# kylc/optik

Hardware: AMD Instinct MI355X
Metric: random-restart IK solves/sec (Panda 7-DoF, 1e-6 tol) (higher is better)
Workload: dtype f64

## Files before the change

### include/optik_hip.h

```cpp
#ifndef OPTIK_HIP_H
#define OPTIK_HIP_H

#include <stdint.h>

#ifdef __cplusplus
extern "C" {
#endif

#define OPTIK_HIP_MAX_DOF 16

enum {
    OPTIK_HIP_OK = 0,
    OPTIK_HIP_EINVAL = -1,
    OPTIK_HIP_EUNSUPPORTED = -2,
    OPTIK_HIP_ENODEVICE = -3,
    OPTIK_HIP_ENOMEM = -4
};

enum { OPTIK_JOINT_FIXED = 0, OPTIK_JOINT_REVOLUTE = 1, OPTIK_JOINT_PRISMATIC = 2 };

enum {
    OPTIK_RES_FAILURE = -1,
    OPTIK_RES_ROUNDOFF_LIMITED = -4,
    OPTIK_RES_FORCED_STOP = -5,
// ... 195 lines not shown
                           const double *d_targets, const double *d_x0, int32_t T, const double *ee_offset7,
                           uint64_t restart_begin, uint64_t restart_end, double deadline_s,
                           int32_t K, double min_dist, const optik_hip_ik_solutions_outputs *out, void *stream);

#define OPTIK_HIP_PATH_MAX_RESTARTS 4096
typedef struct optik_hip_ik_path_outputs {
    double *d_x;
    double *d_f;
    uint64_t *d_idx;
    double *d_key;
    double *d_step;
    double *d_last;
} optik_hip_ik_path_outputs;
int optik_hip_ik_path(optik_hip_chain *chain, const optik_solver_config *cfg, const double *d_targets,
                      const double *d_x0, int32_t P, int32_t L, const double *ee_offset7, uint64_t restart_begin,
                      uint64_t restart_end, uint32_t flags, double deadline_s, double max_step,
                      const optik_hip_ik_path_outputs *out, void *stream);

int optik_hip_set_option(const char *name, long long value);
long long optik_hip_get_option(const char *name);

int optik_hip_ik_host(optik_hip_chain *chain, const optik_solver_config *cfg,
                      const double *targets, const double *x0, int32_t T, const double *ee_offset7,
                      uint64_t restart_begin, uint64_t restart_end, uint32_t flags,
                      double deadline_s, double *win_x, double *win_f, uint64_t *win_idx,
                      double *win_key);

int optik_hip_probe(int32_t op, const double *a, const double *b, int64_t count, double *out);
int optik_hip_probe_math(int32_t op, const double *poses7, int64_t count, double *out);

typedef struct optik_hip_launch_info {
    int32_t grid, block, lds_bytes, tiles;
    float kernel_ms;
} optik_hip_launch_info;
void optik_hip_set_timing(optik_hip_chain *chain, int32_t enabled);
int optik_hip_last_launch(const optik_hip_chain *chain, optik_hip_launch_info *info);
int optik_hip_timing_mean(optik_hip_chain *chain, double *mean_ms, int32_t *count);
int optik_hip_phase_profile(optik_hip_chain *chain, unsigned long long *out8);

#ifdef __cplusplus
}
#endif
#endif
```

### optik_amd/_native.py

```python
from __future__ import annotations

import ctypes as C
import math
import os

_HERE = os.path.dirname(os.path.abspath(__file__))
LIB_PATH = os.path.join(_HERE, "csrc", "liboptik_amd.so")
if os.environ.get("OPTIK_AMD_LIB"):
    LIB_PATH = os.path.abspath(os.environ["OPTIK_AMD_LIB"])

MAX_DOF = 8
IK_EARLY_EXIT = 1
IK_FIND_ANY = 2
IK_RESTART_MAJOR = 4
UINT64_MAX = 0xFFFFFFFFFFFFFFFF

RES_FAILURE, RES_ROUNDOFF, RES_FORCED_STOP, RES_ITER_CAP = -1, -4, -5, -100
RES_STOPVAL, RES_FTOL, RES_XTOL = 2, 3, 4
RANGE_SINGLE_INCLUSIVE, RANGE_NEW_INCLUSIVE = 0, 1


class OptikHipError(RuntimeError):
    pass

# ... 25 lines not shown
                ("d_key", C.c_void_p)]


MAX_SOLUTIONS = 256
MAX_SOLUTION_RESTARTS = 1 << 22


def check_solutions_args(k, min_dist):
    if isinstance(k, bool) or int(k) != k or not 1 <= int(k) <= MAX_SOLUTIONS:
        raise ValueError(f"k must be an integer in 1..{MAX_SOLUTIONS}, got {k!r}")
    min_dist = float(min_dist)
    if not (min_dist >= 0.0 and min_dist != float("inf")):
        raise ValueError(f"min_dist must be finite and >= 0, got {min_dist!r}")
    return int(k), min_dist


class IkPathOutputs(C.Structure):
    _fields_ = [("d_x", C.c_void_p), ("d_f", C.c_void_p), ("d_idx", C.c_void_p), ("d_key", C.c_void_p),
                ("d_step", C.c_void_p), ("d_last", C.c_void_p)]


PATH_MAX_RESTARTS = 4096


def check_max_step(max_step):
    max_step = float(max_step)
    if not max_step >= 0.0:
        raise ValueError(f"max_step must be >= 0 (+inf: no limit), got {max_step!r}")
    return max_step


class LaunchInfo(C.Structure):
    _fields_ = [("grid", C.c_int32), ("block", C.c_int32), ("lds_bytes", C.c_int32),
                ("tiles", C.c_int32), ("kernel_ms", C.c_float)]


_lib = None


def lib():
    global _lib
    if _lib is not None:
        return _lib
    if not os.path.exists(LIB_PATH):
        raise OptikHipError(
            f"{LIB_PATH} is missing: build it with `python -c 'import __graft_entry__ as g; "
            "g.build()'` (hipcc --offload-arch=gfx950).  optik_amd has no CPU fallback.")
    L = C.CDLL(LIB_PATH, mode=C.RTLD_GLOBAL)
    vp, dp, ip = C.c_void_p, C.POINTER(C.c_double), C.POINTER(C.c_int32)
    L.optik_hip_device_count.restype = C.c_int
    L.optik_hip_set_option.argtypes = [C.c_char_p, C.c_longlong]
    L.optik_hip_get_option.argtypes = [C.c_char_p]
    L.optik_hip_get_option.restype = C.c_longlong
    L.optik_hip_last_error.restype = C.c_char_p
    L.optik_hip_chain_create.argtypes = [dp, dp, ip, C.c_int32, dp, dp, C.c_int32, C.POINTER(vp)]
    L.optik_hip_chain_destroy.argtypes = [vp]
    L.optik_hip_chain_num_positions.argtypes = [vp]
    L.optik_hip_chain_set_range_rule.argtypes = [vp, C.c_int32]
    L.optik_hip_chain_range_rule.argtypes = [vp]
    L.optik_hip_eval_batch.argtypes = [vp, C.POINTER(SolverConfigC), dp, dp, vp, C.c_int64, vp, vp, vp]
    L.optik_hip_fk_batch.argtypes = [vp, dp, vp, C.c_int64, vp, vp, vp]
    L.optik_hip_seed_batch.argtypes = [vp, C.c_uint64, C.c_int64, vp, vp]
    L.optik_hip_manip_batch.argtypes = [vp, dp, vp, C.c_int64, vp, vp, vp]
    ip = C.POINTER(C.c_int32)
    L.optik_hip_chain_set_collision_model.argtypes = [vp, ip, dp, dp, C.c_int32, ip, C.c_int32, C.c_double]
    L.optik_hip_chain_set_world.argtypes = [vp, dp, C.c_int32, dp, C.c_int32]
    L.optik_hip_chain_set_world_grid.argtypes = [vp, dp, C.c_double, C.c_int32, C.c_int32, C.c_int32, vp]
# ... 256 lines not shown
```

### optik_amd/csrc/ik_batch_ops.hip

```cpp
#include "diff_ik_lp.hpp"
#include "ik_host.hpp"
#include "ik_jacobian.hpp"

using namespace optik;
using namespace optik::host;
using namespace optik::hostparams;

namespace {

struct EvalLaunch {
    const ChainDev *chain;
    EvalParams ep;
    double target[7];
    const double *q;
    long long B;
    double *f;
    double *g;
};

template <int N, bool TIP>
__global__ __launch_bounds__(256) void eval_batch_kernel(const EvalLaunch a) {
    __shared__ ChainDev sch;
    stage_chain(sch, a.chain);
    const Pose target = load_pose(a.target);
// ... 130 lines not shown
                ++qi;
            } else if (a.types[j] == OPTIK_JOINT_PRISMATIC) {
                const double d = a.q[(size_t)qi * a.B + b];
                local.t = V3{a.axis[j][0] * d, a.axis[j][1] * d, a.axis[j][2] * d};
                ++qi;
            }
            const Pose jt = pose_mul(load_pose(a.origin[j]), local);
            state = pose_mul(state, jt);
        }
        const Pose ee = pose_mul(state, load_pose(a.ee_offset));
        const double p[7] = {ee.t.x, ee.t.y, ee.t.z, ee.q.i, ee.q.j, ee.q.k, ee.q.w};
#pragma unroll
        for (int i = 0; i < 7; ++i) a.pose[(size_t)i * a.B + b] = p[i];
    }
}

struct SeedLaunch {
    uint32_t key[8];
    double lb[MAX_DOF];
    double scale[MAX_DOF];
    unsigned long long first;
    long long count;
    double *q;
};

template <int N>
__global__ __launch_bounds__(256) void seed_batch_kernel(const SeedLaunch a) {
    for (long long b = (long long)blockIdx.x * blockDim.x + threadIdx.x; b < a.count;
         b += (long long)gridDim.x * blockDim.x) {
        double q[N];
        restart_seed<N>(a.key, a.lb, a.scale, a.first + (unsigned long long)b, q);
#pragma unroll
        for (int i = 0; i < N; ++i) a.q[(size_t)i * a.count + b] = q[i];
    }
}

__global__ void probe_kernel(int op, const double *a, const double *b, long long count, double *out) {
    for (long long i = (long long)blockIdx.x * blockDim.x + threadIdx.x; i < count;
         i += (long long)gridDim.x * blockDim.x) {
        double r = 0.0, s, c;
        switch (op) {
        case 0: r = a[i] / b[i]; break;
        case 1: r = __builtin_sqrt(a[i]); break;
        case 2: sincos_dev(a[i], s, c); r = s; break;
        case 3: sincos_dev(a[i], s, c); r = c; break;
        default: r = atan2_q1(a[i], b[i]); break;
        }
        out[i] = r;
    }
}

__global__ void probe_math_kernel(int op, const double *poses, long long count, double *out, int stride) {
    for (long long i = (long long)blockIdx.x * blockDim.x + threadIdx.x; i < count;
         i += (long long)gridDim.x * blockDim.x) {
        const Pose X = load_pose(poses + i * 7);
        double *o = out + i * stride;
        const V3 w = so3_log(X.q);
        if (op == 0) { o[0] = w.x; o[1] = w.y; o[2] = w.z; continue; }
        const RotTerms rt = rot_terms(w);
        const M3 Jr = so3_right_jacobian(rt);
        if (op == 1) {
            for (int r = 0; r < 3; ++r) for (int c = 0; c < 3; ++c) o[r * 3 + c] = Jr.m[r][c];
        } else if (op == 2) {
            const V3 lin = se3_log_linear(rt, X.t);
            o[0] = lin.x; o[1] = lin.y; o[2] = lin.z; o[3] = w.x; o[4] = w.y; o[5] = w.z;
        } else {
            const M3 Q = se3_q_matrix(rt, X.t, Jr);
            for (int r = 0; r < 3; ++r)
                for (int c = 0; c < 3; ++c) {
                    o[r * 6 + c] = Jr.m[r][c];
                    o[r * 6 + 3 + c] = Q.m[r][c];
                    o[(r + 3) * 6 + c] = 0.0;
                    o[(r + 3) * 6 + 3 + c] = Jr.m[r][c];
                }
        }
    }
}

const char *const kPrismaticJacobianMsg =
    "joint_jacobian: prismatic joints are not implemented (the reference panics: kinematics.rs:185 todo!())";

}

extern "C" {

int optik_hip_eval_batch(const optik_hip_chain *ch, const optik_solver_config *cfg, const double *target7,
                         const double *ee_offset7, const double *d_q, int64_t B, double *d_f, double *d_g,
                         void *stream) {
    if (!ch || !cfg || !target7 || !d_q || !d_f || B < 0) return fail(OPTIK_HIP_EINVAL, "bad argument");
    if (B == 0) return 0;
    if (ch->prismatic)
        return fail(OPTIK_HIP_EUNSUPPORTED,
                    "prismatic joints: only forward kinematics is available (the reference's Jacobian panics, kinematics.rs:185)");
    BIND_DEVICE(ch);
    if (ch->wide) {
        WideBatchLaunch w;
        std::memset(&w, 0, sizeof w);
        w.chain = ch->wdev;
        make_eval_params(cfg->linear_weight, cfg->angular_weight, ee_offset7, w.ep);
        std::memcpy(w.target, target7, sizeof w.target);
        w.q = d_q; w.B = B; w.f = d_f; w.g = d_g;
        HIP_TRY(wide_batch_launch(0, grid_for(ch, B, 256, 8), (hipStream_t)stream, w));
        return 0;
    }
    EvalLaunch a;
    a.chain = ch->dev;
    make_eval_params(cfg->linear_weight, cfg->angular_weight, ee_offset7, a.ep);
    std::memcpy(a.target, target7, sizeof a.target);
    a.q = d_q; a.B = B; a.f = d_f; a.g = d_g;
    const int grid = grid_for(ch, B, 256, 8);
#define CALL(NN, TT) hipLaunchKernelGGL((eval_batch_kernel<NN, TT>), dim3(grid), dim3(256), 0, (hipStream_t)stream, a)
    OPTIK_DISPATCH(ch, CALL);
#undef CALL
    HIP_TRY(hipGetLastError());
    return 0;
}
// ... 138 lines not shown
```

### optik_amd/csrc/ik_capi.hip

```cpp
#include <algorithm>
#include <cstdio>
#include <cstdlib>
#include <vector>

#include "ik_host.hpp"

using namespace optik;
using namespace optik::host;
using namespace optik::hostparams;

namespace optik {
namespace host {

thread_local std::string g_err;

static int solve_kernel_from(const char *e) {
    if (!e) return SK_AUTO;
    if (!std::strcmp(e, "quad")) return SK_QUAD;
    if (!std::strcmp(e, "lane64")) return SK_LANE64;
    if (!std::strcmp(e, "general")) return SK_GENERAL;
    return SK_AUTO;
}
Options &opt() {
    static Options o = [] {
// ... 160 lines not shown
    ch->fs_clean = sl.fs_clean_after;
    ch->clean_stream = stream;
}

static int solve_locked(optik_hip_chain *ch, const optik_solver_config *cfg, const double *d_targets,
                        const double *d_x0, int32_t T, const double *ee_offset7, uint64_t restart_begin,
                        uint64_t restart_end, uint32_t flags, double deadline_s, const optik_hip_ik_outputs *out,
                        bool want_sel, bool need_x, bool need_f, hipStream_t stream, bool claim_request,
                        bool *claim_armed, SolvedLaunch *sl) {
    if (!ch || !cfg || !d_targets || !d_x0 || !out || T < 1) return fail(OPTIK_HIP_EINVAL, "bad argument");
    if (restart_end <= restart_begin) return fail(OPTIK_HIP_EINVAL, "empty restart range");
    const int mode = cfg->solution_mode;
    if (mode < OPTIK_MODE_QUALITY || mode > OPTIK_MODE_CONDITION)
        return fail(OPTIK_HIP_EINVAL,
                    "solution_mode must be 1 (Quality), 2 (Speed), 3 (Manipulability) or 4 (Condition)");
    const bool manip = mode == OPTIK_MODE_MANIPULABILITY || mode == OPTIK_MODE_CONDITION;
    const bool coll = ch && ch->coll_S > 0;
    const uint64_t R = restart_end - restart_begin;
    if (restart_end > 1 || restart_begin > 0)
        for (int k = 0; k < ch->n; ++k)
            if (std::isnan(ch->scale[k]))
                return fail(OPTIK_HIP_EINVAL, "random restarts need finite joint limits (reference: random_range panics)");
    if (ch->prismatic)
        return fail(OPTIK_HIP_EUNSUPPORTED,
                    "prismatic joints: only forward kinematics is available (the reference's Jacobian panics, kinematics.rs:185)");

    PlanIn in{};
    in.n = ch->n; in.wide = ch->wide; in.cus = ch->num_cus;
    in.T = T; in.R = R; in.flags = flags; in.mode = mode; in.coll = coll;
    in.solve_kernel = opt().solve_kernel; in.wide_form = opt().wide_form;
    in.claim_request = claim_request; in.have_claim_block = ch->hw_claim != nullptr;
    in.lane_waves = lane_solve_waves_per_cu(); in.quad_waves = quad_solve_waves_per_cu(ch->n);
    in.latency_waves = 4; in.wide_waves = 8;
    const LaunchPlan plan = plan_launch(in);
    if (plan.error == PLAN_TOO_MANY_TILES)
        return fail(OPTIK_HIP_EINVAL, "too many restarts / targets in one launch (2^24 or more selection tiles)");
    const bool early = plan.early, wide_lds = plan.solver == WIDE_LDS, widek = wide_lds || plan.solver == WIDE_HBM;
    const size_t cols = (size_t)plan.cols;

    BIND_DEVICE(ch);
    if (ch->claim_pending && stream != nullptr) { HIP_TRY(hipStreamSynchronize(nullptr)); ch->claim_pending = false; }
    HIP_TRY(ch->tile_recs.reserve((size_t)plan.n_tiles));
    if (!ch->queue) { HIP_TRY(hipMalloc(&ch->queue, sizeof(unsigned long long))); ch->queue_clean = false; }
    if (stream != ch->clean_stream) { ch->queue_clean = false; ch->fs_clean = 0; }
    if (!ch->queue_clean) HIP_TRY(hipMemsetAsync(ch->queue, 0, sizeof(unsigned long long), stream));
    ch->queue_clean = false;
    size_t fs_clean_after = ch->fs_clean;
    if (early) {
        if ((size_t)T > ch->first_success.capacity()) ch->fs_clean = 0;
        HIP_TRY(ch->first_success.reserve((size_t)T));
        if (ch->fs_clean < (size_t)T)
            HIP_TRY(hipMemsetAsync(ch->first_success.get(), 0xff, sizeof(unsigned long long) * (size_t)T, stream));
        fs_clean_after = std::max(ch->fs_clean, (size_t)T);
        ch->fs_clean = 0;
    }
    double *px = out->d_x, *pf = out->d_f, *pk = nullptr;
    need_x = need_x || (want_sel && (manip || coll));
    if (want_sel) {
        const bool need_xf = (!px || !pf) && (need_x || need_f);
        if (cols > ch->tmp_key.capacity()) {
            HIP_TRY(ch->tmp_x.reset());
            HIP_TRY(ch->tmp_f.reset());
            HIP_TRY(ch->tmp_key.reserve(cols));
        }
        if (need_xf) {
            HIP_TRY(ch->tmp_x.reserve(ch->tmp_key.capacity() * (size_t)ch->n));
            HIP_TRY(ch->tmp_f.reserve(ch->tmp_key.capacity()));
        }
        pk = ch->tmp_key.get();
        if (!px && need_x) px = ch->tmp_x.get();
        if (!pf && need_f) pf = ch->tmp_f.get();
    }

    if (widek && !ch->wide) {
        fill_wide_chain(ch->whost, &ch->host.origin[0][0], &ch->host.axis[0][0], ch->host.lb, ch->host.ub, ch->n, ch->tip,
                        ch->scale);
        HIP_TRY(upload_table(&ch->wdev, ch->whost));
    }
    if (plan.solver == WIDE_HBM) HIP_TRY(ch->wide_ws.reserve(wide_ws_doubles_per_wave() * (size_t)plan.grid));

    SolveLaunch a;
    std::memset(&a, 0, sizeof a);
    a.chain = ch->dev;
    make_eval_params(cfg->linear_weight, cfg->angular_weight, ee_offset7, a.ep);
    fill_solve_params(cfg, a.sp, opt().stop_x_legacy != 0);
    std::memcpy(a.key, ch->key, sizeof a.key);
    std::memcpy(a.scale, ch->scale, sizeof a.scale);
    a.wq.next_item = ch->queue;
    a.wq.total_items = (unsigned long long)cols;
    a.wq.n_restarts = R;
    a.wq.restart_begin = restart_begin;
    a.wq.targets = d_targets;
    a.wq.x0 = d_x0;
    a.wq.first_success = early ? ch->first_success.get() : nullptr;
    a.wq.find_any = plan.find_any ? 1 : 0;
    a.wq.restart_major = plan.restart_major ? 1 : 0;
    a.wq.n_targets = (unsigned long long)T;
    a.wq.quality = plan.quality;
    a.wq.lanes = plan.lanes;
    a.wq.out_x = px;
    a.wq.out_f = pf;
    a.wq.out_key = pk;
    a.wq.out_status = out->d_status;
    a.wq.out_evals = out->d_evals;
#ifdef OPTIK_PROFILE
    if (!ch->prof) HIP_TRY(hipMalloc(&ch->prof, 8 * sizeof(unsigned long long)));
    HIP_TRY(hipMemsetAsync(ch->prof, 0, 8 * sizeof(unsigned long long), stream));
    a.wq.prof = ch->prof;
#endif
    if (deadline_s > 0.0) {
        const double khz = ch->wall_clock_khz > 0 ? (double)ch->wall_clock_khz : 100000.0;
        a.deadline_ticks = (unsigned long long)(deadline_s * khz * 1e3);
        if (a.deadline_ticks == 0) a.deadline_ticks = 1;
    }
    if (plan.arm_claim) {
        a.wq.claim = ch->hw_claim;
        a.wq.claim_seq = ++ch->claim_seq;
        if (claim_armed) *claim_armed = true;
        if (stream == nullptr) ch->claim_pending = true;
    }
    const int ev_slot = ch->ev_count % optik_hip_chain::EV_POOL;
    if (ch->timing) {
        if (!ch->ev0[ev_slot]) { HIP_TRY(hipEventCreate(&ch->ev0[ev_slot])); HIP_TRY(hipEventCreate(&ch->ev1[ev_slot])); }
        HIP_TRY(hipEventRecord(ch->ev0[ev_slot], stream));
    }
    int lds = 0;
    if (widek) {
        WideSolveLaunch w;
        std::memset(&w, 0, sizeof w);
        w.chain = ch->wdev;
        w.ep = a.ep; w.sp = a.sp; w.wq = a.wq;
        std::memcpy(w.key, ch->key, sizeof w.key);
        w.deadline_ticks = a.deadline_ticks;
        w.ws = ch->wide_ws.get();
        lds = wide_lds ? wide_lds_bytes() : (int)sizeof(WideChainDev);
        HIP_TRY(wide_solve_launch(plan.grid, stream, w, wide_lds, opt().wide_form != 2));
    } else if (plan.solver == LANE) {
        HIP_TRY(lane_solve_launch(ch->n, ch->tip, plan.grid, stream, a, &lds));
    } else {
        HIP_TRY(quad_solve_launch(ch->n, ch->tip, plan.grid, stream, a, &lds, plan.solver == QUAD_LATENCY));
    }
    HIP_TRY(hipGetLastError());
    if (ch->timing) { HIP_TRY(hipEventRecord(ch->ev1[ev_slot], stream)); ch->ev_count += 1; }
    if (manip && pk)
        if (int rc = manip_key_launch(ch, mode, ee_offset7, px, pk, cols, stream)) return rc;
    if (coll && pk)
        if (int rc = collision_key_launch(ch, ee_offset7, px, pk, cols, stream)) return rc;
    ch->last.grid = plan.grid; ch->last.block = WAVE; ch->last.lds_bytes = lds; ch->last.tiles = plan.n_tiles;

    sl->px = px; sl->pf = pf; sl->pk = pk;
    sl->R = R;
    sl->tiles_per_target = plan.tiles_per_target;
    sl->cols = cols;
    sl->fs_clean_after = fs_clean_after;
    sl->early = early;
    return 0;
}

static int ik_batch_locked(optik_hip_chain *ch, const optik_solver_config *cfg, const double *d_targets,
                           const double *d_x0, int32_t T, const double *ee_offset7, uint64_t restart_begin,
                           uint64_t restart_end, uint32_t flags, double deadline_s, const optik_hip_ik_outputs *out,
                           void *stream_v, bool claim_request = false, bool *claim_armed = nullptr) {
    if (claim_armed) *claim_armed = false;
    if (!out) return fail(OPTIK_HIP_EINVAL, "bad argument");
    hipStream_t stream = (hipStream_t)stream_v;
    const bool want_win = out->d_win_x || out->d_win_f || out->d_win_idx || out->d_win_key;
    SolvedLaunch sl;
    if (int rc = solve_locked(ch, cfg, d_targets, d_x0, T, ee_offset7, restart_begin, restart_end, flags, deadline_s,
                              out, want_win, out->d_win_x != nullptr, out->d_win_f != nullptr, stream, claim_request,
                              claim_armed, &sl))
        return rc;
    BIND_DEVICE(ch);
    if (want_win) {
        SelectLaunch s;
        std::memset(&s, 0, sizeof s);
        s.out_key = sl.pk; s.out_x = sl.px; s.out_f = sl.pf;
        s.tile_recs = ch->tile_recs.get();
        s.tiles_per_target = (int)sl.tiles_per_target;
        s.tile = SEL_TILE;
        s.n = ch->n;
        s.restart_begin = restart_begin;
// ... 103 lines not shown
        PathSelectLaunch s;
        std::memset(&s, 0, sizeof s);
        s.out_key = sl.pk; s.out_x = sl.px; s.out_f = sl.pf;
        s.seed = seed;
        s.carry = ch->path_carry.get();
        s.last = l + 1 == L ? out->d_last : nullptr;
        s.n = n;
        s.filter = filter ? 1 : 0;
        s.max_step = max_step;
        s.restart_begin = restart_begin;
        s.n_restarts = sl.R;
        s.ld = sl.cols;
        s.x = out->d_x ? out->d_x + w * (size_t)n : nullptr;
        s.f = out->d_f ? out->d_f + w : nullptr;
        s.idx = out->d_idx ? (unsigned long long *)out->d_idx + w : nullptr;
        s.key = out->d_key ? out->d_key + w : nullptr;
        s.step = out->d_step ? out->d_step + w : nullptr;
        s.reset_queue = ch->queue;
        s.reset_fs = sl.early ? ch->first_success.get() : nullptr;
        HIP_TRY(path_select_launch(s, P, stream));
        words_put_back(ch, sl, stream);
    }
    return 0;
}

static int *option_slot(const char *name) {
    Options &o = opt();
    if (!name) return nullptr;
    if (!std::strcmp(name, "solve_kernel")) return &o.solve_kernel;
    if (!std::strcmp(name, "wide_form")) return &o.wide_form;
    if (!std::strcmp(name, "range_rule")) return &o.range_rule;
    if (!std::strcmp(name, "stop_x_legacy")) return &o.stop_x_legacy;
    if (!std::strcmp(name, "grid_cap")) return &o.grid_cap;
    return nullptr;
}
int optik_hip_set_option(const char *name, long long value) {
    int *slot = option_slot(name);
    if (!slot) return fail(OPTIK_HIP_EINVAL, "unknown option");
    if (slot == &opt().grid_cap && (value < 0 || value > 0x7fffffffll))
        return fail(OPTIK_HIP_EINVAL, "grid_cap must be >= 0 (0: the device's cap)");
    *slot = (int)value;
    return 0;
}
long long optik_hip_get_option(const char *name) {
    const int *slot = option_slot(name);
    return slot ? (long long)*slot : -1;
}

int optik_hip_ik_host(optik_hip_chain *ch, const optik_solver_config *cfg, const double *targets,
                      const double *x0, int32_t T, const double *ee_offset7, uint64_t restart_begin,
                      uint64_t restart_end, uint32_t flags, double deadline_s, double *win_x, double *win_f,
                      uint64_t *win_idx, double *win_key) {
    if (!ch || !cfg || !targets || !x0 || T < 1) return fail(OPTIK_HIP_EINVAL, "bad argument");
    std::lock_guard<std::mutex> host_lock(ch->host_mu);
    BIND_DEVICE(ch);
    const int n = ch->n;
    const size_t n_in = (size_t)(7 + n) * (size_t)T, n_out = (size_t)(n + 3) * (size_t)T;
    std::unique_lock<std::mutex> launch_lock(ch->mu);
    if (n_in + n_out > ch->hw_dev.capacity() || 2 * (n_in + n_out) > ch->hw_pin.capacity()) {
        if (ch->claim_pending) { (void)hipStreamSynchronize(nullptr); ch->claim_pending = false; }
        HIP_TRY(ch->hw_dev.reserve(n_in + n_out));
        HIP_TRY(ch->hw_pin.reserve(2 * (n_in + n_out)));
    }
    const bool zero_copy = T <= 16;
    double *pin = ch->hw_pin.get();
    if (zero_copy) {
        pin += (ch->hw_flip & 1u) * (ch->hw_pin.capacity() / 2);
        ch->hw_flip ^= 1u;
    } else if (ch->claim_pending) {
        HIP_TRY(hipStreamSynchronize(nullptr));
        ch->claim_pending = false;
    }
    double *io = zero_copy ? pin : ch->hw_dev.get();
// ... 107 lines not shown
```

### optik_amd/csrc/ik_host.hpp

```cpp
#pragma once

#include <hip/hip_runtime.h>

#include <cmath>
#include <cstring>
#include <mutex>
#include <string>

#include "../../include/optik_hip.h"
#include "device_buf.hpp"
#include "device_scope.hpp"
#include "ik_grid.hpp"
#include "ik_host_params.hpp"
#include "ik_launch.hpp"
#include "ik_launch_plan.hpp"
#include "ik_wide_launch.hpp"

namespace optik {
namespace coll {
struct ModelDev;
}
namespace host {

static_assert(PLAN_EARLY_EXIT == OPTIK_HIP_IK_EARLY_EXIT && PLAN_FIND_ANY == OPTIK_HIP_IK_FIND_ANY
// ... 53 lines not shown
struct PathSelectLaunch {
    const double *out_key;
    const double *out_x;
    const double *out_f;
    const double *seed;
    double *carry;
    double *last;
    int n;
    int filter;
    double max_step;
    unsigned long long restart_begin;
    unsigned long long n_restarts;
    size_t ld;
    double *x;
    double *f;
    unsigned long long *idx;
    double *key;
    double *step;
    unsigned long long *reset_queue;
    unsigned long long *reset_fs;
};
hipError_t path_select_launch(const PathSelectLaunch &s, int P, hipStream_t stream);

int manip_key_launch(const optik_hip_chain *ch, int mode, const double *ee_offset7, const double *x, double *key,
                     size_t cols, hipStream_t stream);

int collision_key_launch(const optik_hip_chain *ch, const double *ee_offset7, const double *x, double *key,
                         size_t cols, hipStream_t stream);

int motion_reserve(optik_hip_chain *ch, long long segments);
int motion_key_launch(const optik_hip_chain *ch, const double *ee_offset7, const double *seed, const double *x,
                      double *key, int P, size_t R, int filter, double max_step, hipStream_t stream);

struct Options {
    int solve_kernel = SK_AUTO;
    int wide_form = WF_LDS;
    int range_rule = OPTIK_HIP_RANGE_SINGLE_INCLUSIVE;
    int stop_x_legacy = 0;
    int grid_cap = 0;
};
Options &opt();

extern thread_local std::string g_err;
inline int fail(int code, const std::string &msg) {
    g_err = msg;
    return code;
}

#define HIP_TRY(expr)                                                                   \
    do {                                                                                \
        hipError_t e_ = (expr);                                                         \
        if (e_ != hipSuccess)                                                           \
            return ::optik::host::fail(OPTIK_HIP_ENODEVICE, std::string(#expr) + ": " + hipGetErrorString(e_)); \
    } while (0)

inline int ensure_device() {
    int n = 0;
    hipError_t e = hipGetDeviceCount(&n);
    if (e != hipSuccess || n <= 0)
        return fail(OPTIK_HIP_ENODEVICE, std::string("no HIP device available: ")
                                             + (e == hipSuccess ? "device count is 0" : hipGetErrorString(e)));
    return 0;
}

#define BIND_DEVICE(CH)                                                                 \
    optik::DeviceScope dev_scope_((CH)->device_id);                                     \
    if (!dev_scope_.ok()) return ::optik::host::fail(OPTIK_HIP_ENODEVICE, "hipSetDevice(" + std::to_string((CH)->device_id) + ") failed")

#define OPTIK_N_RANGE_MSG "this kernel is built for 1 <= n <= 8 revolute joints"
#define OPTIK_DISPATCH_ONE(NN, CALL)                                                   \
    if (!done_ && n_ == NN) {                                                          \
        if (tip_) { CALL(NN, true); } else { CALL(NN, false); }                        \
// ... 25 lines not shown
    bool wide = false;
    optik::WideChainDev whost;
    optik::WideChainDev *wdev = nullptr;
    optik::DeviceBuf<double> wide_ws;
    int device_id = 0;
    bool prismatic = false;
    int n_joints = 0;
    int32_t types[optik::MAX_JOINTS] = {};
    double axis_all[optik::MAX_JOINTS][3] = {};
    std::mutex mu;
    std::mutex host_mu;
    optik::DeviceBuf<optik::host::TileRec> tile_recs;
    optik::DeviceBuf<unsigned long long> first_success;
    optik::DeviceBuf<unsigned long long> sol_pick;
    optik::DeviceBuf<double> path_carry;
    int coll_S = 0, coll_P = 0, coll_groups = 0;
    double coll_margin = 0.0;
    optik::coll::ModelDev *coll_dev = nullptr;
    optik::DeviceBuf<uint16_t> coll_orig;
    optik::DeviceBuf<double> world_dev;
    int world_Ms = 0, world_Mb = 0;
    optik::DeviceBuf<float> grid_dev;
    int grid_n[3] = {0, 0, 0};
    double grid_origin[3] = {0.0, 0.0, 0.0};
    double grid_inv = 0.0;
    double motion_h = 0.0;
    optik::DeviceBuf<unsigned char> motion_ws;
    optik::DeviceBuf<unsigned char> roadmap_ws;
    optik::DeviceBuf<unsigned char> shortcut_ws;
    bool queue_clean = false;
    size_t fs_clean = 0;
    hipStream_t clean_stream = nullptr;
    optik::DeviceBuf<double> tmp_x, tmp_f, tmp_key;
    unsigned long long *queue = nullptr;
    unsigned long long *prof = nullptr;
    optik::DeviceBuf<double> hw_dev;
    optik::PinnedBuf<double> hw_pin;
    unsigned long long *hw_claim = nullptr;
    hipEvent_t claim_done = nullptr;
    unsigned long long claim_seq = 0;
    bool claim_pending = false;
    unsigned hw_flip = 0;
    int timing = 0;
    static constexpr int EV_POOL = 256;
    hipEvent_t ev0[EV_POOL] = {}, ev1[EV_POOL] = {};
    int ev_count = 0;
    optik_hip_launch_info last{};
    int num_cus = 0;
    int wall_clock_khz = 0;
    optik::DeviceBuf<unsigned char> edt_ws;
    optik::DeviceBuf<float> depth_ws;
};

namespace optik {
namespace host {

inline int grid_for(const optik_hip_chain *ch, long long work, int block, int per_cu) {
    const long long cap = (long long)(ch->num_cus > 0 ? ch->num_cus : 256) * per_cu;
    return stride_grid(work > 0 ? (unsigned long long)work : 0ull, block, cap, opt().grid_cap);
}

}
}
```

### optik_amd/csrc/ik_lane64.hpp

```cpp
#pragma once

#include "ik_lane.hpp"
#include "ik_solve.hpp"
#include "ik_nnls_quad.hpp"

namespace optik {

template <int N>
struct Lane64Geom {
    static constexpr int NG = N * (N + 1) / 2;
    static constexpr int REC = NG + 2 * N;
    OPTIK_DEV static constexpr int g(int i, int j) { return i * N - (i * (i - 1)) / 2 + (j - i); }
    OPTIK_DEV static constexpr int hlo(int i) { return NG + i; }
    OPTIK_DEV static constexpr int hhi(int i) { return NG + N + i; }
    static constexpr int META = NnlsQuadGeom<N>::XS + 2 * N;
    static_assert(NnlsQuadGeom<N>::XS + 2 * N + 3 <= NnlsQuadGeom<N>::STRIDE, "three spare doubles per block");
};

}
#include "ik_nnls_first.hpp"
namespace optik {

#ifndef OPTIK_LANE_FIRST_PASS_MIN
#define OPTIK_LANE_FIRST_PASS_MIN 16
#endif
#ifndef OPTIK_LANE_WARM_START
#define OPTIK_LANE_WARM_START 1
#endif
#ifndef OPTIK_LANE_FIRST_PASS
#define OPTIK_LANE_FIRST_PASS 1
#endif

template <int N>
constexpr int lane64_block_lds() { return nnls_quad_wave_lds<N>(); }
template <int N>
constexpr int lane64_rec_lds() { return Lane64Geom<N>::REC * 64; }

#ifndef OPTIK_LANE_CLASSES
#define OPTIK_LANE_CLASSES 8
#endif
constexpr int LANE64_CLASSES = OPTIK_LANE_CLASSES;
#ifndef OPTIK_LANE_PIPE
#define OPTIK_LANE_PIPE 1
#endif
#ifndef LANE64_MAX_RUNNING
#define LANE64_MAX_RUNNING 14
#endif
#ifndef OPTIK_LANE_RESERVE
#define OPTIK_LANE_RESERVE 8
#endif
#ifndef OPTIK_LANE_KEEP_TARGET
#define OPTIK_LANE_KEEP_TARGET 1
#endif
#ifndef OPTIK_LANE_REFILL
#define OPTIK_LANE_REFILL 4
#endif

template <int N, class Expand, class ReadBack>
struct Lane64Pipe {
    static constexpr bool on = true;
    static constexpr bool warm_start = true;
    static constexpr int MAX_RUNNING = LANE64_MAX_RUNNING;
    int n_prob, next, hold;
    int qi, ql, lane, rank;
    bool has, got;
    double *bk;
    int *lor, *where;
    Expand *expand_fn;
    ReadBack *read_fn;
    OPTIK_DEV bool more() const { return next < n_prob; }
    template <bool WARM>
    OPTIK_DEV bool event(bool idle, int mode, double rn, int passes, double *wst, int &wj) {
        wj = 0;
        const bool fin = idle && hold >= 0;
        if (wave_any(fin)) {
            if (fin && ql == 0) {
                bk[Lane64Geom<N>::META] = (double)mode;
                bk[Lane64Geom<N>::META + 1] = rn;
                bk[Lane64Geom<N>::META + 2] = (double)passes;
                where[hold] = 0x100 | qi;
            }
            lds_sync();
// ... 17 lines not shown
            if (live) hold = pr;
        }
        return live;
    }
};

template <int N, bool TIP>
OPTIK_DEV void lane64_wave(const ChainDev &ch, const EvalParams &ep, const SolveParams &sp, const uint32_t (&key)[8],
                           const double (&scale)[MAX_DOF], const WorkQueue &wq,
                           double *nnls_lds ,
                           double *rec_lds , int *lor_lds ,
                           int *where_lds ) {
    typedef Lane64Geom<N> G;
    constexpr int NL = N * (N + 1) / 2;
    constexpr int NS = (N > 4) ? 2 : 1;
    constexpr int CS = NnlsQuadGeom<N>::CS;
    static_assert(N <= 7, "the throughput form of chains with at most seven joints");
    const double alfmin = 0.1;
    const int lane = (int)(threadIdx.x & 63u);
    double x[N], x0[N], g[N], s[N], l[NL];
    double xbest[N], xprev[N];
    double f = 0.0, f0 = 0.0, t0 = 0.0, h3 = 0.0, alpha = 1.0;
    double minf = __builtin_huge_val(), fprev = __builtin_huge_val();
    int ireset = 0, line = 0, nevals = 0;
    int pred = 1;
    bool first = true;
    bool again = false;
    Pose target;
    unsigned long long item = 0, index = 0;
    unsigned tslot = OPTIK_LANE_KEEP_TARGET ? ~0u : 0u;
    bool active = false, want = lane < wq.lanes;
#if OPTIK_LANE_RESERVE > 0
    unsigned long long rbase = 0, rend = 0;
    unsigned long long pend = 0;
    bool r_pending = false;
    bool dry = false;
#endif
#pragma unroll
    for (int i = 0; i < N; ++i) { x[i] = 0.0; x0[i] = 0.0; g[i] = 0.0; s[i] = 0.0; xbest[i] = 0.0; xprev[i] = 0.0; }
#pragma unroll
    for (int i = 0; i < NL; ++i) l[i] = 0.0;
    target.t = V3{0, 0, 0};
    target.q = Q4{0, 0, 0, 1};

#ifdef OPTIK_PROFILE
    unsigned long long lp_[8] = {0, 0, 0, 0, 0, 0, 0, 0};
    unsigned long long lt_ = __builtin_readcyclecounter();
#define LANE_PROF(slot) do { const unsigned long long n_ = __builtin_readcyclecounter(); lp_[slot] += n_ - lt_; lt_ = n_; } while (0)
#else
#define LANE_PROF(slot)
#endif
    for (;;) {
        const unsigned n_want = (unsigned)__popcll(__ballot(want));
        if (n_want >= (unsigned)(wq.lanes < OPTIK_LANE_REFILL ? wq.lanes : OPTIK_LANE_REFILL) || (n_want > 0 && !wave_any(active))) {
#if OPTIK_LANE_RESERVE > 0
            unsigned long long it;
            {
                if (r_pending) { rbase = __shfl(pend, 0); rend = rbase + OPTIK_LANE_RESERVE; r_pending = false; }
                const unsigned long long wm = __ballot(want);
                const unsigned rank = (unsigned)__popcll(wm & ((1ull << lane) - 1ull));
                const unsigned long long have = rend - rbase;
                const unsigned long long take = n_want < have ? n_want : have;
                it = rbase + rank;
                rbase += take;
                if (wave_any(want && rank >= take)) {
                    const unsigned long long it2 = fetch_items(wq.next_item, want && rank >= take);
                    if (rank >= take) it = it2;
                }
                dry = dry || wave_any(want && it >= wq.total_items);
            }
#else
            const unsigned long long it = fetch_items(wq.next_item, want);
#endif
            if (want) {
                want = false;
                if (it < wq.total_items) {
                    unsigned long long r;
#if OPTIK_LANE_KEEP_TARGET
                    const unsigned tprev = tslot;
#endif
                    if (wq.restart_major) { r = it / wq.n_targets; tslot = (unsigned)(it - r * wq.n_targets); }
                    else { tslot = (unsigned)(it / wq.n_restarts); r = it - (unsigned long long)tslot * wq.n_restarts; }
                    item = (unsigned long long)tslot * wq.n_restarts + r;
                    index = wq.restart_begin + r;
#if OPTIK_LANE_KEEP_TARGET
                    if (tslot != tprev) target = load_pose(wq.targets + (size_t)tslot * 7);
#else
                    target = load_pose(wq.targets + (size_t)tslot * 7);
#endif
                    restart_seed<N>(key, ch.lb, scale, index, x);
                    if (index == 0) {
                        const double *x0p = wq.x0 + (size_t)tslot * N;
#pragma unroll
                        for (int i = 0; i < N; ++i) x[i] = x0p[i];
                    }
#pragma unroll
                    for (int i = 0; i < N; ++i) { xbest[i] = x[i]; xprev[i] = x[i]; x0[i] = x[i]; s[i] = 0.0; g[i] = 0.0; }
                    f = 0.0; f0 = 0.0; t0 = 0.0; h3 = 0.0; alpha = 1.0;
                    minf = __builtin_huge_val(); fprev = __builtin_huge_val();
                    ireset = 0; line = 0; nevals = 0; pred = 1;
                    first = true;
                    again = false;
                    active = true;
                }
            }
        }
#if OPTIK_LANE_RESERVE > 0
        if (!r_pending && rbase == rend && !dry) {
            if (lane == 0) pend = atomicAdd(wq.next_item, (unsigned long long)OPTIK_LANE_RESERVE);
            r_pending = true;
        }
#endif
        if (!wave_any(active)) break;
        LANE_PROF(0);

        int32_t ret = 0;
        if (active) {
            bool stop = false;
            if (wq.first_success) {
                const unsigned long long fs = __hip_atomic_load(wq.first_success + tslot, __ATOMIC_RELAXED,
                                                                __HIP_MEMORY_SCOPE_AGENT);
                stop = wq.find_any ? (fs != ~0ull) : (fs < index);
            }
// ... 380 lines not shown
```

### optik_amd/csrc/ik_launch_plan.hpp

```cpp
#pragma once

#include <algorithm>
#include <cstdint>

namespace optik {
namespace host {

constexpr int WAVE = 64;
constexpr int QUADS_PER_WAVE_HOST = 16;
constexpr int SEL_TILE = 4096;

enum : int { SK_AUTO = 0, SK_QUAD = 1, SK_LANE64 = 2, SK_GENERAL = 3 };
enum : int { WF_LDS = 0, WF_HBM = 1 };
constexpr uint32_t PLAN_EARLY_EXIT = 1u, PLAN_FIND_ANY = 2u, PLAN_RESTART_MAJOR = 4u;
constexpr int PLAN_MODE_SPEED = 2;

struct PlanIn {
    int n;
    bool wide;
    int cus;
    int32_t T;
    uint64_t R;
    uint32_t flags;
    int mode;
    bool coll;
    int solve_kernel;
    int wide_form;
    bool claim_request;
    bool have_claim_block;
    int lane_waves, quad_waves, latency_waves, wide_waves;
};

enum PlanSolver : int { QUAD_LATENCY, QUAD, LANE, WIDE_LDS, WIDE_HBM };
enum PlanError : int { PLAN_OK = 0, PLAN_TOO_MANY_TILES };

struct LaunchPlan {
    PlanError error;
    PlanSolver solver;
    bool early;
    bool find_any;
    bool quality;
    bool restart_major;
    bool arm_claim;
    int lanes;
    long long resident;
    int grid;
    uint64_t tiles_per_target;
    int n_tiles;
    uint64_t cols;
};

inline LaunchPlan plan_launch(const PlanIn &in) {
    LaunchPlan p{};
    p.tiles_per_target = (in.R + SEL_TILE - 1) / SEL_TILE;
    const uint64_t n_tiles64 = p.tiles_per_target * (uint64_t)in.T;
    if (n_tiles64 * 256ull >= (1ull << 32)) { p.error = PLAN_TOO_MANY_TILES; return p; }
    p.n_tiles = (int)n_tiles64;
    p.cols = (uint64_t)in.T * in.R;
    const long long cols = (long long)p.cols, T = in.T;

    p.early = (in.flags & PLAN_EARLY_EXIT) && in.mode == PLAN_MODE_SPEED && !in.coll;
    p.find_any = p.early && (in.flags & PLAN_FIND_ANY);
    p.restart_major = (in.flags & PLAN_RESTART_MAJOR) != 0;
    p.quality = in.mode != PLAN_MODE_SPEED;
    const bool early_rm = p.early && p.restart_major;

    const bool widek = in.wide || in.solve_kernel == SK_GENERAL;
    const bool lane_able = !widek && in.n <= 7 && in.solve_kernel != SK_QUAD;
    const bool lane_forced = lane_able && in.solve_kernel == SK_LANE64;
    const long long cus = in.cus > 0 ? in.cus : 256;
    const bool quad_latency = !widek && cols <= cus * in.latency_waves && !lane_forced;
    const bool lanek = lane_able && !quad_latency && (lane_forced || (cols >= cus * in.lane_waves * WAVE && !early_rm));
    p.solver = widek ? (in.wide_form != WF_HBM ? WIDE_LDS : WIDE_HBM) : lanek ? LANE : quad_latency ? QUAD_LATENCY : QUAD;
    const long long cap = cus * (widek ? in.wide_waves : lanek ? in.lane_waves : quad_latency ? in.latency_waves : in.quad_waves);
    const long long per_wave_max = (widek || lanek) ? WAVE : QUADS_PER_WAVE_HOST;

    const long long inflight = 8;
    p.resident = cols;
    if (early_rm && p.resident > T * inflight)
        p.resident = std::max(T * inflight, std::min(p.resident, std::max(2 * cap, T * 32)));
    const long long lanes = p.solver == WIDE_LDS ? 1 : std::clamp((p.resident + cap - 1) / cap, 1ll, per_wave_max);
    p.lanes = (int)lanes;
    p.grid = (int)std::min((p.resident + lanes - 1) / lanes, cap);
    p.arm_claim = in.claim_request && in.have_claim_block && (p.solver == QUAD || p.solver == QUAD_LATENCY) && p.find_any
                  && in.T == 1;
    return p;
}

}
}
```

### optik_amd/csrc/ik_solve.hpp

```cpp
#pragma once

#include "ik_slsqp.hpp"

namespace optik {

enum : int32_t {
    RES_FAILURE = -1,
    RES_ROUNDOFF_LIMITED = -4,
    RES_FORCED_STOP = -5,
    RES_ITER_CAP = -100,
    RES_STOPVAL_REACHED = 2,
    RES_FTOL_REACHED = 3,
    RES_XTOL_REACHED = 4,
};

constexpr int MAX_EVALS_CAP = 100000;
constexpr unsigned REFILL_BATCH = 8;

#ifdef OPTIK_PROFILE
#define OPTIK_PROF_DECL unsigned long long prof_[8] = {0, 0, 0, 0, 0, 0, 0, 0}; unsigned long long prof_t_ = 0
#define OPTIK_PROF_BEGIN() prof_t_ = __builtin_readcyclecounter()
#define OPTIK_PROF_END(slot) prof_[slot] += __builtin_readcyclecounter() - prof_t_
#define OPTIK_PROF_COUNT(slot, n) prof_[slot] += (n)
#define OPTIK_PROF_SUB_BEGIN() const unsigned long long prof_s_ = __builtin_readcyclecounter()
// ... 74 lines not shown
    static_assert(N <= 8, "one ChaCha block per restart");
    uint32_t blk[16];
    chacha8_block(key, 0, index, blk);
#pragma unroll
    for (int k = 0; k < N; ++k) {
        const uint64_t bits = (uint64_t)blk[2 * k] | ((uint64_t)blk[2 * k + 1] << 32);
        q[k] = uniform_inclusive(lb[k], scale[k], bits);
    }
}


struct WorkQueue {
    unsigned long long *next_item;
    unsigned long long total_items;
    unsigned long long n_restarts;
    unsigned long long restart_begin;
    const double *targets;
    const double *x0;
    unsigned long long *first_success;
    int find_any;
    int restart_major;
    unsigned long long n_targets;
    unsigned long long deadline;
    int quality;
    int lanes;
    double *out_x;
    double *out_f;
    double *out_key;
    int32_t *out_status;
    int32_t *out_evals;
    unsigned long long *prof;
    unsigned long long *claim;
    unsigned long long claim_seq;
};

OPTIK_DEV unsigned long long fetch_items(unsigned long long *counter, bool want) {
    const unsigned long long mask = __ballot(want);
    const unsigned n = (unsigned)__popcll(mask);
    unsigned long long base = 0;
    if (n) {
        const int leader = __ffsll((long long)mask) - 1;
        const int lane = (int)(threadIdx.x & 63u);
        if (lane == leader) base = atomicAdd(counter, (unsigned long long)n);
        base = __shfl(base, leader, 64);
    }
    const unsigned rank = (unsigned)__popcll(mask & ((1ull << (threadIdx.x & 63u)) - 1ull));
    return base + rank;
}

}
```

### optik_amd/device.py

```python
from __future__ import annotations

import ctypes as C

import numpy as np
import torch

from . import _native as nat


def _stream_ptr():
    return C.c_void_p(torch.cuda.current_stream().cuda_stream)


def _ptr(t):
    return C.c_void_p(t.data_ptr()) if t is not None else C.c_void_p(None)


def _dp(a):
    return a.ctypes.data_as(C.POINTER(C.c_double))


class HipChain:

    def __init__(self, types, origins, axes, lb, ub, device="cuda:0"):
# ... 565 lines not shown
        o.d_key, o.d_step, o.d_last = _ptr(bufs.get("key")), _ptr(bufs.get("step")), _ptr(bufs.get("last"))
        ee = np.ascontiguousarray(ee_offset7, dtype=np.float64) if ee_offset7 is not None else None
        nat.check(nat.lib().optik_hip_ik_path(
            self._h, C.byref(cfg), _ptr(targets), _ptr(x0), P, L, _dp(ee) if ee is not None else None, b, e,
            int(flags), float(deadline_s), max_step, C.byref(o), _stream_ptr()))
        return bufs

    def ik_host(self, cfg, targets, x0, restart_begin, restart_end, flags=0, deadline_s=0.0, ee_offset7=None):
        targets = np.ascontiguousarray(targets, dtype=np.float64)
        x0 = np.ascontiguousarray(x0, dtype=np.float64)
        T = targets.shape[0]
        assert targets.shape == (T, 7) and x0.shape == (T, self.n)
        win_x = np.zeros((T, self.n)); win_f = np.zeros(T); win_key = np.zeros(T)
        win_idx = np.zeros(T, dtype=np.uint64)
        ee = np.ascontiguousarray(ee_offset7, dtype=np.float64) if ee_offset7 is not None else None
        nat.check(nat.lib().optik_hip_ik_host(
            self._h, C.byref(cfg), _dp(targets), _dp(x0), T, _dp(ee) if ee is not None else None,
            int(restart_begin), int(restart_end), int(flags), float(deadline_s), _dp(win_x), _dp(win_f),
            win_idx.ctypes.data_as(C.POINTER(C.c_uint64)), _dp(win_key)))
        return dict(win_x=win_x, win_f=win_f, win_idx=win_idx.astype(np.int64), win_key=win_key)

    def set_timing(self, enabled=True):
        nat.lib().optik_hip_set_timing(self._h, 1 if enabled else 0)

    def timing_mean(self):
        ms, cnt = C.c_double(0.0), C.c_int32(0)
        nat.check(nat.lib().optik_hip_timing_mean(self._h, C.byref(ms), C.byref(cnt)))
        return ms.value, cnt.value

    def last_launch(self):
        info = nat.LaunchInfo()
        nat.check(nat.lib().optik_hip_last_launch(self._h, C.byref(info)))
        return dict(grid=info.grid, block=info.block, lds_bytes=info.lds_bytes, tiles=info.tiles,
                    kernel_ms=info.kernel_ms)


def probe(op, a, b=None):
    a = np.ascontiguousarray(a, dtype=np.float64)
    b = np.ascontiguousarray(b if b is not None else a, dtype=np.float64)
    out = np.empty_like(a)
    nat.check(nat.lib().optik_hip_probe(int(op), _dp(a), _dp(b), a.size, _dp(out)))
    return out


_MATH_STRIDE = {0: 3, 1: 9, 2: 6, 3: 36}


def probe_math(op, poses7):
    p = np.ascontiguousarray(poses7, dtype=np.float64).reshape(-1, 7)
    out = np.empty((p.shape[0], _MATH_STRIDE[int(op)]), dtype=np.float64)
    nat.check(nat.lib().optik_hip_probe_math(int(op), _dp(p), p.shape[0], _dp(out)))
    if op == 1:
        return out.reshape(-1, 3, 3)
    if op == 3:
        return out.reshape(-1, 6, 6)
    return out
```

Baseline: 35.56 million.

## Precompute restart seeds into a shared table and carry item index decomposition

When the lane solver runs with multiple targets, a pre-pass kernel computes each restart's ChaCha-based seed once into a device table. Solver lanes then read the row instead of regenerating the seed per (target, restart) item. The lane work loop also carries the quotient/remainder of the item index incrementally, avoiding a 64-bit division per fetched item. This costs an extra kernel launch, table memory (capped by a new option) and global loads in exchange for less per-item ALU work.

```diff
diff --git a/include/optik_hip.h b/include/optik_hip.h
--- a/include/optik_hip.h
+++ b/include/optik_hip.h
@@ -251,6 +251,8 @@
 typedef struct optik_hip_launch_info {
     int32_t grid, block, lds_bytes, tiles;
     float kernel_ms;
+    int32_t reserved;
+    int64_t seed_rows;
 } optik_hip_launch_info;
 void optik_hip_set_timing(optik_hip_chain *chain, int32_t enabled);
 int optik_hip_last_launch(const optik_hip_chain *chain, optik_hip_launch_info *info);
diff --git a/optik_amd/_native.py b/optik_amd/_native.py
--- a/optik_amd/_native.py
+++ b/optik_amd/_native.py
@@ -81,7 +81,7 @@
 
 class LaunchInfo(C.Structure):
     _fields_ = [("grid", C.c_int32), ("block", C.c_int32), ("lds_bytes", C.c_int32),
-                ("tiles", C.c_int32), ("kernel_ms", C.c_float)]
+                ("tiles", C.c_int32), ("kernel_ms", C.c_float), ("reserved", C.c_int32), ("seed_rows", C.c_int64)]
 
 
 _lib = None
diff --git a/optik_amd/csrc/ik_batch_ops.hip b/optik_amd/csrc/ik_batch_ops.hip
--- a/optik_amd/csrc/ik_batch_ops.hip
+++ b/optik_amd/csrc/ik_batch_ops.hip
@@ -186,6 +186,18 @@
         restart_seed<N>(a.key, a.lb, a.scale, a.first + (unsigned long long)b, q);
 #pragma unroll
         for (int i = 0; i < N; ++i) a.q[(size_t)i * a.count + b] = q[i];
+    }
+}
+
+template <int N>
+__global__ __launch_bounds__(256) void seed_table_kernel(const SeedLaunch a) {
+    static_assert(N <= SEED_ROW, "a row holds the seed");
+    for (long long b = (long long)blockIdx.x * blockDim.x + threadIdx.x; b < a.count;
+         b += (long long)gridDim.x * blockDim.x) {
+        double q[N];
+        restart_seed<N>(a.key, a.lb, a.scale, a.first + (unsigned long long)b, q);
+#pragma unroll
+        for (int i = 0; i < N; ++i) a.q[(size_t)b * SEED_ROW + i] = q[i];
     }
 }
 
@@ -236,6 +248,26 @@
 
 }
 
+namespace optik {
+namespace host {
+
+int seed_table_launch(const optik_hip_chain *ch, uint64_t first, uint64_t rows, double *d_table, hipStream_t stream) {
+    SeedLaunch a;
+    std::memcpy(a.key, ch->key, sizeof a.key);
+    std::memcpy(a.lb, ch->host.lb, sizeof a.lb);
+    std::memcpy(a.scale, ch->scale, sizeof a.scale);
+    a.first = first; a.count = (long long)rows; a.q = d_table;
+    const int grid = grid_for(ch, (long long)rows, 256, 8);
+#define CALL(NN, TT) hipLaunchKernelGGL((seed_table_kernel<NN>), dim3(grid), dim3(256), 0, stream, a)
+    OPTIK_DISPATCH(ch, CALL);
+#undef CALL
+    HIP_TRY(hipGetLastError());
+    return 0;
+}
+
+}
+}
+
 extern "C" {
 
 int optik_hip_eval_batch(const optik_hip_chain *ch, const optik_solver_config *cfg, const double *target7,
diff --git a/optik_amd/csrc/ik_capi.hip b/optik_amd/csrc/ik_capi.hip
--- a/optik_amd/csrc/ik_capi.hip
+++ b/optik_amd/csrc/ik_capi.hip
@@ -216,6 +216,8 @@
     in.claim_request = claim_request; in.have_claim_block = ch->hw_claim != nullptr;
     in.lane_waves = lane_solve_waves_per_cu(); in.quad_waves = quad_solve_waves_per_cu(ch->n);
     in.latency_waves = 4; in.wide_waves = 8;
+    in.grid_cap = opt().grid_cap;
+    in.seed_table_cap = opt().seed_table_cap > 0 ? (uint64_t)opt().seed_table_cap : 0;
     const LaunchPlan plan = plan_launch(in);
     if (plan.error == PLAN_TOO_MANY_TILES)
         return fail(OPTIK_HIP_EINVAL, "too many restarts / targets in one launch (2^24 or more selection tiles)");
@@ -262,6 +264,7 @@
         HIP_TRY(upload_table(&ch->wdev, ch->whost));
     }
     if (plan.solver == WIDE_HBM) HIP_TRY(ch->wide_ws.reserve(wide_ws_doubles_per_wave() * (size_t)plan.grid));
+    if (plan.seed_table) HIP_TRY(ch->seed_table.reserve((size_t)plan.seed_rows * SEED_ROW));
 
     SolveLaunch a;
     std::memset(&a, 0, sizeof a);
@@ -320,6 +323,10 @@
         lds = wide_lds ? wide_lds_bytes() : (int)sizeof(WideChainDev);
         HIP_TRY(wide_solve_launch(plan.grid, stream, w, wide_lds, opt().wide_form != 2));
     } else if (plan.solver == LANE) {
+        if (plan.seed_table) {
+            if (int rc = seed_table_launch(ch, restart_begin, plan.seed_rows, ch->seed_table.get(), stream)) return rc;
+            a.wq.seeds = ch->seed_table.get();
+        }
         HIP_TRY(lane_solve_launch(ch->n, ch->tip, plan.grid, stream, a, &lds));
     } else {
         HIP_TRY(quad_solve_launch(ch->n, ch->tip, plan.grid, stream, a, &lds, plan.solver == QUAD_LATENCY));
@@ -331,6 +338,7 @@
     if (coll && pk)
         if (int rc = collision_key_launch(ch, ee_offset7, px, pk, cols, stream)) return rc;
     ch->last.grid = plan.grid; ch->last.block = WAVE; ch->last.lds_bytes = lds; ch->last.tiles = plan.n_tiles;
+    ch->last.seed_rows = (int64_t)plan.seed_rows;
 
     sl->px = px; sl->pf = pf; sl->pk = pk;
     sl->R = R;
@@ -500,6 +508,7 @@
     if (!std::strcmp(name, "range_rule")) return &o.range_rule;
     if (!std::strcmp(name, "stop_x_legacy")) return &o.stop_x_legacy;
     if (!std::strcmp(name, "grid_cap")) return &o.grid_cap;
+    if (!std::strcmp(name, "seed_table_cap")) return &o.seed_table_cap;
     return nullptr;
 }
 int optik_hip_set_option(const char *name, long long value) {
@@ -507,6 +516,8 @@
     if (!slot) return fail(OPTIK_HIP_EINVAL, "unknown option");
     if (slot == &opt().grid_cap && (value < 0 || value > 0x7fffffffll))
         return fail(OPTIK_HIP_EINVAL, "grid_cap must be >= 0 (0: the device's cap)");
+    if (slot == &opt().seed_table_cap && (value < 0 || value > 0x7fffffffll))
+        return fail(OPTIK_HIP_EINVAL, "seed_table_cap must be in 0 .. 2^31 - 1 bytes (0: no table)");
     *slot = (int)value;
     return 0;
 }
diff --git a/optik_amd/csrc/ik_host.hpp b/optik_amd/csrc/ik_host.hpp
--- a/optik_amd/csrc/ik_host.hpp
+++ b/optik_amd/csrc/ik_host.hpp
@@ -109,12 +109,15 @@
 int motion_key_launch(const optik_hip_chain *ch, const double *ee_offset7, const double *seed, const double *x,
                       double *key, int P, size_t R, int filter, double max_step, hipStream_t stream);
 
+int seed_table_launch(const optik_hip_chain *ch, uint64_t first, uint64_t rows, double *d_table, hipStream_t stream);
+
 struct Options {
     int solve_kernel = SK_AUTO;
     int wide_form = WF_LDS;
     int range_rule = OPTIK_HIP_RANGE_SINGLE_INCLUSIVE;
     int stop_x_legacy = 0;
     int grid_cap = 0;
+    int seed_table_cap = SEED_TABLE_CAP_BYTES;
 };
 Options &opt();
 
@@ -206,6 +209,7 @@
     size_t fs_clean = 0;
     hipStream_t clean_stream = nullptr;
     optik::DeviceBuf<double> tmp_x, tmp_f, tmp_key;
+    optik::DeviceBuf<double> seed_table;
     unsigned long long *queue = nullptr;
     unsigned long long *prof = nullptr;
     optik::DeviceBuf<double> hw_dev;
diff --git a/optik_amd/csrc/ik_lane64.hpp b/optik_amd/csrc/ik_lane64.hpp
--- a/optik_amd/csrc/ik_lane64.hpp
+++ b/optik_amd/csrc/ik_lane64.hpp
@@ -48,6 +48,9 @@
 #endif
 #ifndef OPTIK_LANE_RESERVE
 #define OPTIK_LANE_RESERVE 8
+#endif
+#ifndef OPTIK_LANE_CARRY
+#define OPTIK_LANE_CARRY 1
 #endif
 #ifndef OPTIK_LANE_KEEP_TARGET
 #define OPTIK_LANE_KEEP_TARGET 1
@@ -131,6 +134,9 @@
     bool active = false, want = lane < wq.lanes;
 #if OPTIK_LANE_RESERVE > 0
     unsigned long long rbase = 0, rend = 0;
+#if OPTIK_LANE_CARRY
+    unsigned long long b_hi = 0, b_lo = 0;
+#endif
     unsigned long long pend = 0;
     bool r_pending = false;
     bool dry = false;
@@ -152,34 +158,60 @@
     for (;;) {
         const unsigned n_want = (unsigned)__popcll(__ballot(want));
         if (n_want >= (unsigned)(wq.lanes < OPTIK_LANE_REFILL ? wq.lanes : OPTIK_LANE_REFILL) || (n_want > 0 && !wave_any(active))) {
+            const unsigned long long per = wq.restart_major ? wq.n_targets : wq.n_restarts;
+            unsigned long long it, hi = 0, lo = 0;
 #if OPTIK_LANE_RESERVE > 0
-            unsigned long long it;
             {
-                if (r_pending) { rbase = __shfl(pend, 0); rend = rbase + OPTIK_LANE_RESERVE; r_pending = false; }
+                if (r_pending) {
+                    rbase = __shfl(pend, 0);
+                    rend = rbase + OPTIK_LANE_RESERVE;
+                    r_pending = false;
+#if OPTIK_LANE_CARRY
+                    b_hi = rbase / per;
+                    b_lo = rbase - b_hi * per;
+#endif
+                }
                 const unsigned long long wm = __ballot(want);
                 const unsigned rank = (unsigned)__popcll(wm & ((1ull << lane) - 1ull));
                 const unsigned long long have = rend - rbase;
                 const unsigned long long take = n_want < have ? n_want : have;
                 it = rbase + rank;
+#if OPTIK_LANE_CARRY
+                if (want && rank < take) {
+                    hi = b_hi;
+                    lo = b_lo + rank;
+                    while (lo >= per) { lo -= per; ++hi; }
+                }
+                b_lo += take;
+                while (b_lo >= per) { b_lo -= per; ++b_hi; }
+#endif
                 rbase += take;
                 if (wave_any(want && rank >= take)) {
                     const unsigned long long it2 = fetch_items(wq.next_item, want && rank >= take);
                     if (rank >= take) it = it2;
-                }
+#if OPTIK_LANE_CARRY
+                    if (rank >= take) { hi = it2 / per; lo = it2 - hi * per; }
+#endif
+                }
+#if !OPTIK_LANE_CARRY
+                hi = it / per;
+                lo = it - hi * per;
+#endif
                 dry = dry || wave_any(want && it >= wq.total_items);
             }
 #else
-            const unsigned long long it = fetch_items(wq.next_item, want);
+            it = fetch_items(wq.next_item, want);
+            hi = it / per;
+            lo = it - hi * per;
 #endif
             if (want) {
                 want = false;
                 if (it < wq.total_items) {
-                    unsigned long long r;
 #if OPTIK_LANE_KEEP_TARGET
                     const unsigned tprev = tslot;
 #endif
-                    if (wq.restart_major) { r = it / wq.n_targets; tslot = (unsigned)(it - r * wq.n_targets); }
-                    else { tslot = (unsigned)(it / wq.n_restarts); r = it - (unsigned long long)tslot * wq.n_restarts; }
+                    const unsigned long long r = wq.restart_major ? hi : lo;
+                    tslot = (unsigned)(wq.restart_major ? lo : hi);
                     item = (unsigned long long)tslot * wq.n_restarts + r;
                     index = wq.restart_begin + r;
 #if OPTIK_LANE_KEEP_TARGET
@@ -187,7 +219,13 @@
 #else
                     target = load_pose(wq.targets + (size_t)tslot * 7);
 #endif
-                    restart_seed<N>(key, ch.lb, scale, index, x);
+                    if (wq.seeds) {
+                        const double *const row = wq.seeds + (size_t)SEED_ROW * r;
+#pragma unroll
+                        for (int i = 0; i < N; ++i) x[i] = row[i];
+                    } else {
+                        restart_seed<N>(key, ch.lb, scale, index, x);
+                    }
                     if (index == 0) {
                         const double *x0p = wq.x0 + (size_t)tslot * N;
 #pragma unroll
diff --git a/optik_amd/csrc/ik_launch_plan.hpp b/optik_amd/csrc/ik_launch_plan.hpp
--- a/optik_amd/csrc/ik_launch_plan.hpp
+++ b/optik_amd/csrc/ik_launch_plan.hpp
@@ -9,6 +9,8 @@
 constexpr int WAVE = 64;
 constexpr int QUADS_PER_WAVE_HOST = 16;
 constexpr int SEL_TILE = 4096;
+constexpr int SEED_ROW_BYTES = 64;
+constexpr int SEED_TABLE_CAP_BYTES = 64 << 20;
 
 enum : int { SK_AUTO = 0, SK_QUAD = 1, SK_LANE64 = 2, SK_GENERAL = 3 };
 enum : int { WF_LDS = 0, WF_HBM = 1 };
@@ -29,6 +31,8 @@
     bool claim_request;
     bool have_claim_block;
     int lane_waves, quad_waves, latency_waves, wide_waves;
+    int grid_cap;
+    uint64_t seed_table_cap;
 };
 
 enum PlanSolver : int { QUAD_LATENCY, QUAD, LANE, WIDE_LDS, WIDE_HBM };
@@ -48,6 +52,9 @@
     uint64_t tiles_per_target;
     int n_tiles;
     uint64_t cols;
+    bool seed_table;
+    uint64_t seed_rows;
+    uint64_t seed_bytes;
 };
 
 inline LaunchPlan plan_launch(const PlanIn &in) {
@@ -72,7 +79,8 @@
     const bool quad_latency = !widek && cols <= cus * in.latency_waves && !lane_forced;
     const bool lanek = lane_able && !quad_latency && (lane_forced || (cols >= cus * in.lane_waves * WAVE && !early_rm));
     p.solver = widek ? (in.wide_form != WF_HBM ? WIDE_LDS : WIDE_HBM) : lanek ? LANE : quad_latency ? QUAD_LATENCY : QUAD;
-    const long long cap = cus * (widek ? in.wide_waves : lanek ? in.lane_waves : quad_latency ? in.latency_waves : in.quad_waves);
+    long long cap = cus * (widek ? in.wide_waves : lanek ? in.lane_waves : quad_latency ? in.latency_waves : in.quad_waves);
+    if (in.grid_cap >= 1) cap = std::min(cap, (long long)in.grid_cap);
     const long long per_wave_max = (widek || lanek) ? WAVE : QUADS_PER_WAVE_HOST;
 
     const long long inflight = 8;
@@ -84,6 +92,9 @@
     p.grid = (int)std::min((p.resident + lanes - 1) / lanes, cap);
     p.arm_claim = in.claim_request && in.have_claim_block && (p.solver == QUAD || p.solver == QUAD_LATENCY) && p.find_any
                   && in.T == 1;
+    p.seed_table = p.solver == LANE && in.T >= 2 && in.R <= in.seed_table_cap / SEED_ROW_BYTES;
+    p.seed_rows = p.seed_table ? in.R : 0;
+    p.seed_bytes = p.seed_rows * SEED_ROW_BYTES;
     return p;
 }
 
diff --git a/optik_amd/csrc/ik_solve.hpp b/optik_amd/csrc/ik_solve.hpp
--- a/optik_amd/csrc/ik_solve.hpp
+++ b/optik_amd/csrc/ik_solve.hpp
@@ -130,7 +130,9 @@
     unsigned long long *prof;
     unsigned long long *claim;
     unsigned long long claim_seq;
+    const double *seeds;
 };
+constexpr int SEED_ROW = 8;
 
 OPTIK_DEV unsigned long long fetch_items(unsigned long long *counter, bool want) {
     const unsigned long long mask = __ballot(want);
diff --git a/optik_amd/device.py b/optik_amd/device.py
--- a/optik_amd/device.py
+++ b/optik_amd/device.py
@@ -621,7 +621,7 @@
         info = nat.LaunchInfo()
         nat.check(nat.lib().optik_hip_last_launch(self._h, C.byref(info)))
         return dict(grid=info.grid, block=info.block, lds_bytes=info.lds_bytes, tiles=info.tiles,
-                    kernel_ms=info.kernel_ms)
+                    kernel_ms=info.kernel_ms, seed_rows=info.seed_rows)
 
 
 def probe(op, a, b=None):
```

Result: slower. 34.58 million (-2.7%).
